# PRBonn/semantic_suma

Measured on AMD Instinct MI355X. Metric: scans_per_sec, higher is better.
Workload: dtype f32; 1 GPU; BASELINE configs[1]: synthetic KITTI-like sequence, 64x2048 range images, semantic-weighted ICP (10 GN iterations + stats pass) + surfel fusion, one sequence per GPU, scans resident in HBM, processScan called scan after scan by the native host loop (suma_pipeline_run_scans); timed after 300 untimed scans of the same sequence (5 warm-up + pre-roll to the steady map size: 1016645 surfels at the star; preroll_scans=300, map_surfels_start=1016645, map_surfels_end=2308753, parallelism=single GPU

## Files before the change

semantic_suma_amd/csrc/k_update.hip:

```cpp
#include <cstddef>
#include <cstring>

#include "suma_internal.h"

#define ST_AGG 1u
#define ST_INC 2u

__device__ __forceinline__ unsigned long long st_pack(uint32_t epoch, uint32_t flag, uint32_t value) {
  return ((unsigned long long)epoch << 34) | ((unsigned long long)flag << 32) | value;
}

struct Pair {
  uint32_t a, x;
};
__device__ __forceinline__ void lookback_publish(unsigned long long* __restrict__ status,
                                                 unsigned long long* __restrict__ group, uint32_t tile, uint32_t agg,
                                                 uint32_t epoch, uint32_t aggx = 0) {
  __hip_atomic_store(&status[tile], st_pack(epoch, ST_AGG, (aggx << 16) | agg), __ATOMIC_RELAXED, __HIP_MEMORY_SCOPE_AGENT);
  __hip_atomic_fetch_add(&group[tile >> 6], (1ull << 56) | ((unsigned long long)aggx << 32) | (unsigned long long)agg,
                         __ATOMIC_RELAXED, __HIP_MEMORY_SCOPE_AGENT);
}
#define SUMA_SPIN_LIMIT (1u << 26)
#ifndef LB_BATCH
#define LB_BATCH 4
#endif
template <bool PAIR>
__device__ Pair lookback_collect2(unsigned long long* __restrict__ status, unsigned long long* __restrict__ group,
                                  uint32_t tile, uint32_t epoch, int lane, uint32_t* __restrict__ fault) {
  const uint32_t g = tile >> 6;
  uint32_t sum = 0, sumx = 0;
  bool timed_out = false;
  const uint32_t j = tile & 63u;
  const bool own = (uint32_t)lane < j;
  unsigned long long ws = 0;
  if (own) ws = __hip_atomic_load(&status[(g << 6) + lane], __ATOMIC_RELAXED, __HIP_MEMORY_SCOPE_AGENT);
  for (uint32_t base = 0; base < g; base += 64u * LB_BATCH) {
    unsigned long long w[LB_BATCH];
#pragma unroll
    for (int q = 0; q < LB_BATCH; ++q) {
      const uint32_t gi = base + (uint32_t)q * 64u + (uint32_t)lane;
      w[q] = gi < g ? __hip_atomic_load(&group[gi], __ATOMIC_RELAXED, __HIP_MEMORY_SCOPE_AGENT) : (64ull << 56);
    }
#pragma unroll
    for (int q = 0; q < LB_BATCH; ++q) {
      const uint32_t gi = base + (uint32_t)q * 64u + (uint32_t)lane;
      uint32_t spins = 0;
      while ((uint32_t)(w[q] >> 56) != 64u && ++spins < SUMA_SPIN_LIMIT)
        w[q] = __hip_atomic_load(&group[gi], __ATOMIC_RELAXED, __HIP_MEMORY_SCOPE_AGENT);
      timed_out |= (spins >= SUMA_SPIN_LIMIT);
      sum += (uint32_t)(w[q] & 0xffffffffull);
      if (PAIR) sumx += (uint32_t)(w[q] >> 32) & 0xffffffu;
    }
  }
  if (own) {
    uint32_t spins = 0;
    while (((uint32_t)(ws >> 34) != (epoch & 0x3fffffffu) || ((ws >> 32) & 3ull) == 0) && ++spins < SUMA_SPIN_LIMIT)
      ws = __hip_atomic_load(&status[(g << 6) + lane], __ATOMIC_RELAXED, __HIP_MEMORY_SCOPE_AGENT);
    timed_out |= (spins >= SUMA_SPIN_LIMIT);
    sum += (uint32_t)(ws & 0xffffull);
    if (PAIR) sumx += (uint32_t)(ws >> 16) & 0xffffu;
  }
  if (timed_out) {
    atomicOr(fault, 8u);
    atomicOr(fault + (offsetof(DevState, fault_site) - offsetof(DevState, overflow)) / 4, 0x2u);
  }
  Pair r;
  r.a = (uint32_t)__builtin_amdgcn_readlane((int)wave_inclusive_scan(sum), 63);
  r.x = PAIR ? (uint32_t)__builtin_amdgcn_readlane((int)wave_inclusive_scan(sumx), 63) : 0u;
  return r;
}
__device__ __forceinline__ uint32_t lookback_collect(unsigned long long* __restrict__ status,
                                                     unsigned long long* __restrict__ group, uint32_t tile, uint32_t epoch,
                                                     int lane, uint32_t* __restrict__ fault) {
  return lookback_collect2<false>(status, group, tile, epoch, lane, fault).a;
}
__device__ uint32_t lookback_prefix(unsigned long long* __restrict__ status, unsigned long long* __restrict__ group,
                                    uint32_t tile, uint32_t agg, uint32_t epoch, int lane, uint32_t* __restrict__ fault) {
  if (lane == 0) lookback_publish(status, group, tile, agg, epoch);
  return lookback_collect(status, group, tile, epoch, lane, fault);
}

struct BlockRank {
  uint32_t rank, total;
};
#define TILE_WAVES (SUMA_TILE / 64)
__device__ __forceinline__ BlockRank block_rank(bool flag, uint32_t* s_wave ) {
  const int lane = threadIdx.x & 63, wave = threadIdx.x >> 6;
  const unsigned long long ball = __ballot(flag);
  const uint32_t below = __popcll(ball & ((1ull << lane) - 1ull));
  if (lane == 0) s_wave[wave] = __popcll(ball);
  __syncthreads();
  uint32_t off = 0, tot = 0;
#pragma unroll
  for (int w = 0; w < (int)TILE_WAVES; ++w) {
    uint32_t cnt = s_wave[w];
    if (w < wave) off += cnt;
    tot += cnt;
  }
  BlockRank r;
  r.rank = off + below;
  r.total = tot;
  return r;
}

__device__ __forceinline__ void block_rank2(bool fa, bool fb, uint32_t* s_wa, uint32_t* s_wb, BlockRank* ra, BlockRank* rb) {
  const int lane = threadIdx.x & 63, wave = threadIdx.x >> 6;
  const unsigned long long ba = __ballot(fa), bb = __ballot(fb);
  const unsigned long long lo = (1ull << lane) - 1ull;
  if (lane == 0) {
    s_wa[wave] = __popcll(ba);
    s_wb[wave] = __popcll(bb);
  }
  __syncthreads();
  uint32_t offa = 0, tota = 0, offb = 0, totb = 0;
#pragma unroll
  for (int w = 0; w < (int)TILE_WAVES; ++w) {
    const uint32_t ca = s_wa[w], cb = s_wb[w];
    if (w < wave) {
      offa += ca;
      offb += cb;
    }
    tota += ca;
    totb += cb;
  }
  ra->rank = offa + __popcll(ba & lo);
  ra->total = tota;
  rb->rank = offb + __popcll(bb & lo);
  rb->total = totb;
}

__device__ __forceinline__ bool is_finaliser(uint32_t failing_ticket, uint32_t ntiles) {
  return failing_ticket == ntiles + gridDim.x - 1;
}
__device__ __forceinline__ void finalise_tickets(DevState* ds, unsigned long long* group_next, uint32_t group_words) {
  for (uint32_t gi = threadIdx.x; gi < group_words; gi += blockDim.x) group_next[gi] = 0;
  if (threadIdx.x == 0) ds->ticket = 0;
}

__device__ __forceinline__ void commit_extraction(DevState* ds, CacheSlot* slots, uint32_t slot, uint32_t base,
                                                  uint32_t arena_cap, uint32_t n) {
  if (n > SUMA_EXTRACT_CAPACITY) {
    n = SUMA_EXTRACT_CAPACITY;
    atomicOr(&ds->overflow, 4u);
  }
  if ((uint64_t)base + n > arena_cap) {
    n = arena_cap - base;
    atomicOr(&ds->overflow, 2u);
  }
  slots[slot].offset = base;
  slots[slot].count = n;
  ds->cache_used = base + n;
  ds->n_extracted = n;
}

__device__ __forceinline__ void write_pose_entry(float* poses, float* poses_inv, uint32_t pose_idx, const m4& pose) {
  float inv[16];
  rigid_inverse_dev(pose.m, inv);
  for (int i = 0; i < 16; ++i) {
    poses[16 * (size_t)pose_idx + i] = pose.m[i];
    poses_inv[16 * (size_t)pose_idx + i] = inv[i];
  }
}
__global__ void __launch_bounds__(256)
    k8_radius(const float4* __restrict__ V, const float4* __restrict__ N, K8Out o, uint32_t P, DevState* ds,
              float* poses, float* poses_inv, uint32_t pose_idx, m4 pose, const float4* __restrict__ Sem) {
  uint32_t pix = blockIdx.x * blockDim.x + threadIdx.x;
  if (pix >= P) return;
  if (pix == 0) {
    ds->n_updated = 0;
    ds->n_data = 0;
    ds->n_kept_updated = 0;
    ds->n_kept_data = 0;
    write_pose_entry(poses, poses_inv, pose_idx, pose);
  }
  k8_pixel(o, pix, V[pix], N[pix], Sem[pix]);
}
__global__ void k8_pose_only(float* poses, float* poses_inv, uint32_t pose_idx, m4 pose) {
  if (threadIdx.x == 0 && blockIdx.x == 0) write_pose_entry(poses, poses_inv, pose_idx, pose);
}

struct UpdArgs {
  const suma_surfel* in;
  suma_surfel* out;
  DevState* ds;
  const float* poses;
  const float* poses_inv;
  unsigned long long* zbuf;
  unsigned long long* status;
  unsigned long long *group, *group_next;
  uint32_t group_words;
  uint32_t epoch;
  const float4 *V, *N, *Sem;
  const float4* radius_conf;
  const float4* pixrec;
  uint8_t* integrated;
  uint32_t* index_map;
  proj_t q;
  m4 pose, inv_pose;
  int32_t timestamp;
  uint32_t max_surfels;
  float confidence_threshold, map_max_distance, update_angle_thresh;
  float p_stable, p_unstable, log_prior, log_unstable, sigma_angle, sigma_distance, max_weight;
  int32_t use_stability, unstable_age, confidence_mode, active_timestamps, weighting_scheme, averaging_scheme,
      update_always;
  float cx, cy, extent;
  uint8_t* ex_flags;
  float ex_cx, ex_cy, ex_extent;
  suma_surfel* x_arena;
  CacheSlot* x_slots;
  uint32_t x_cap, x_slot;
  float* poses_w;
  float* poses_inv_w;
  uint32_t pose_idx;
  int write_pose;
};

__device__ __forceinline__ void load_pose(const float* __restrict__ table, int32_t idx, float* M) {
  const float4* src = reinterpret_cast<const float4*>(table + 16 * (size_t)idx);
#pragma unroll
  for (int k = 0; k < 4; ++k) {
    float4 col = src[k];
    M[4 * k] = col.x;
    M[4 * k + 1] = col.y;
    M[4 * k + 2] = col.z;
    M[4 * k + 3] = col.w;
  }
}

__global__ void __launch_bounds__(256) k7_indexmap(UpdArgs a) {
  const uint32_t S = a.ds->n_surfels;
  const float4* __restrict__ sf = reinterpret_cast<const float4*>(a.in);
  for (uint32_t i = blockIdx.x * blockDim.x + threadIdx.x; i < S; i += gridDim.x * blockDim.x) {
    float4 s0 = sf[4 * (size_t)i], s1 = sf[4 * (size_t)i + 1];
    float count = sf[4 * (size_t)i + 2].w;
    float Ps[16], M[16];
    load_pose(a.poses, (int32_t)count, Ps);
    m4_mul(a.inv_pose.m, Ps, M);
    v3 p = m4_point(M, xyz(s0)), n = m4_dir(M, xyz(s1));
    float lp = len3(p);
    if (!(dot3(n, divs3(neg3(p), lp)) > 0.01f)) continue;
    v3 pr = project01(a.q, p);
    float fx = sdm_floor(pr.x * a.q.width), fy = sdm_floor(pr.y * a.q.height);
    if (!(fx >= 0.0f && fx < a.q.width && fy >= 0.0f && fy < a.q.height)) continue;
    float zn = 2.0f * pr.z - 1.0f;
    if (!(zn >= -1.0f && zn <= 1.0f)) continue;
    unsigned long long key = ((unsigned long long)depth24(0.5f * zn + 0.5f) << 32) | i;
    zbuf_min(&a.zbuf[(size_t)(int32_t)fy * a.q.W + (size_t)(int32_t)fx], key);
  }
}

__device__ __forceinline__ v3 slerp3(v3 v0, v3 v1, float weight) {
  float omega = sdm_acos(dot3(normalize3(v0), normalize3(v1)));
  float so = sdm_sin(omega);
  if (!(so > 0.0f)) return v0;
  float eta = 1.0f / so;
  float w0 = eta * sdm_sin(weight * omega);
  float w1 = eta * sdm_sin((1.0f - weight) * omega);
  return add3(scale3(w0, v0), scale3(w1, v1));
}

struct Surfel4 {
  float4 a, b, c, d;
};

__device__ __forceinline__ bool in_active_area(const UpdArgs& a, const Surfel4& s, bool* in_tile) {
  float Ps[16];
  load_pose(a.poses, (int32_t)s.c.w, Ps);
  v3 pos = m4_point(Ps, xyz(s.a));
  *in_tile = !(sdm_abs(pos.x - a.ex_cx) > a.ex_extent || sdm_abs(pos.y - a.ex_cy) > a.ex_extent);
  if ((int32_t)__float_as_uint(s.c.x) < 0) return false;
  if (sdm_abs(pos.x - a.cx) > a.extent || sdm_abs(pos.y - a.cy) > a.extent) return false;
  return true;
}

__device__ __forceinline__ void store_surfel(suma_surfel* out, uint32_t idx, const Surfel4& s) {
  float4* o = reinterpret_cast<float4*>(out) + 4 * (size_t)idx;
  store_stream(o, s.a);
  store_stream(o + 1, s.b);
  store_stream(o + 2, s.c);
  store_stream(o + 3, s.d);
}

struct K9Pre {
  v3 old_position, old_normal;
  float imz;
  int32_t tx, ty;
  uint32_t rpix;
  bool in_tex, visible, inside;
};
struct K9Rec {
  float4 dv, dn, dx;
  unsigned long long k7key;
};

__device__ __forceinline__ K9Pre k9_prepare(const UpdArgs& a, const Surfel4& in) {
  K9Pre p;
  const int32_t creation_timestamp = (int32_t)in.c.w;
  float Ps[16];
  load_pose(a.poses, creation_timestamp, Ps);
  p.old_position = m4_point(Ps, xyz(in.a));
  p.old_normal = m4_dir(Ps, xyz(in.b));
  const v3 vertex = m4_point(a.inv_pose.m, p.old_position);
  const v3 normal = normalize3(m4_dir(a.inv_pose.m, p.old_normal));
  p.visible = dot3(normal, divs3(neg3(vertex), len3(vertex))) > 0.0f;
  const v3 pr = project01(a.q, vertex);
  const float imx = sdm_floor(pr.x * a.q.width) + 0.5f, imy = sdm_floor(pr.y * a.q.height) + 0.5f;
  p.imz = pr.z;
  p.in_tex = (imx >= 0.0f && imx < a.q.width && imy >= 0.0f && imy < a.q.height);
  p.tx = p.in_tex ? (int32_t)sdm_floor(imx) : -1;
  p.ty = p.in_tex ? (int32_t)sdm_floor(imy) : -1;
  p.rpix = (uint32_t)max(p.ty, 0) * (uint32_t)a.q.W + (uint32_t)max(p.tx, 0);
  p.inside = (imx < a.q.width && imy < a.q.height && p.imz < 1.0f) && !(imx < 0.0f && imy < 0.0f && p.imz < 0.0f);
  return p;
}

__device__ __forceinline__ K9Rec k9_gather(const UpdArgs& a, const K9Pre& p) {
  K9Rec r;
  const float4* __restrict__ rec = a.pixrec + 4 * (size_t)p.rpix;
  r.dv = rec[0];
  r.dn = rec[1];
  r.dx = rec[2];
  r.k7key = a.zbuf[p.rpix];
  return r;
}

__device__ __forceinline__ bool k9_finish(const UpdArgs& a, uint32_t i, const Surfel4& in, const K9Pre& p,
                                          const K9Rec& g, Surfel4& o, int32_t* mark_pix) {
  const int32_t timestamp = a.timestamp;
  const int32_t W = a.q.W;
  const int32_t surfel_age = timestamp - (int32_t)__float_as_uint(in.c.x);
  const int32_t creation_timestamp = (int32_t)in.c.w;
  const v3 old_position = p.old_position, old_normal = p.old_normal;
  const float old_radius = in.a.w, old_confidence = in.b.w, old_weight = in.c.z;

  bool keep = true;
  if (old_confidence < a.confidence_threshold && a.use_stability) keep = (surfel_age < a.unstable_age);
  o = in;
  o.c.y = pack_rgb(0.3f, 0.3f, 0.3f);

  float4 dv = g.dv, dn = g.dn, dx = g.dx;
  if (!p.in_tex) dv = dn = dx = f4(0.f, 0.f, 0.f, 0.f);
  const float4 ds = f4(dx.x, 0.f, 0.f, dx.y), rc = f4(dx.z, 0.f, 0.f, 0.f);
  const unsigned long long k7key = g.k7key;
  const bool valid = (dv.w > 0.5f) && (dn.w > 0.5f);
  const float imz = p.imz;
  const int32_t tx = p.tx, ty = p.ty;

  float penalty = 0.0f;
  float update_confidence = a.log_prior;
  bool mark = false;

  if (valid && p.inside && p.visible) {
    const float data_label = ds.x * 255.0f, data_prob = ds.w;
    const float model_label = in.d.x * 255.0f, model_prob = in.d.w;
    if (sdm_round(data_label) != sdm_round(model_label)) {
      if (is_dynamic_label(model_label)) penalty = 1.0f;
    }
    const v3 v = xyz(dv), n = xyz(dn);
    const v3 v_global = m4_point(a.pose.m, v);
    const v3 n_global = normalize3(m4_dir(a.pose.m, n));
    const v3 view_dir = divs3(neg3(v), len3(v));
    const float distance = sdm_abs(dot3(old_normal, sub3(v_global, old_position)));
    const float angle = len3(cross3(n_global, old_normal));
    const float new_radius = rc.x, new_confidence = rc.y;

    if ((distance < a.map_max_distance) && (angle < a.update_angle_thresh)) {
      mark = true;
      const float confidence = old_confidence + new_confidence;
      o.b.w = confidence;
      o.c.x = __uint_as_float((uint32_t)timestamp);
      float avg_radius = fmin_(new_radius, old_radius);
      avg_radius = fmax_(avg_radius, 0.0f);
      o.a.w = avg_radius;
      keep = true;
      o.c.y = pack_rgb(0.0f, 0.7f, 0.0f);
      o.c.w = (float)creation_timestamp;

      float pst = a.p_stable;
      if (a.confidence_mode == 1 || a.confidence_mode == 3)
        pst *= sdm_exp((-angle * angle) / (a.sigma_angle * a.sigma_angle));
      if (a.confidence_mode == 2 || a.confidence_mode == 3)
        pst *= sdm_exp((-distance * distance) / (a.sigma_distance * a.sigma_distance));
      pst = fclamp(pst, a.p_unstable, 1.0f);
      update_confidence = sdm_log(pst / (1.0f - pst));

      if ((new_radius < old_radius && timestamp - creation_timestamp < a.active_timestamps) || a.update_always) {
        float w1 = 0.9f, w2 = 0.1f;
        if (a.weighting_scheme > 0) {
          w1 = old_weight;
          w2 = 1.0f;
          if (a.weighting_scheme == 2) w2 = dot3(n, view_dir);
          o.c.z = fmin_(a.max_weight, w1 + w2);
          float sum = w1 + w2;
          w1 /= sum;
          w2 /= sum;
        }
        v3 avg_position = add3(scale3(w1, old_position), scale3(w2, v_global));
        v3 avg_normal = slerp3(old_normal, n_global, w1);
        float avg_prob;
        if (sdm_round(data_label) != sdm_round(model_label))
          avg_prob = w1 * model_prob + w2 * (1.0f - data_prob);
        else
          avg_prob = w1 * model_prob + w2 * data_prob;
        o.d.w = avg_prob;
        if (a.averaging_scheme == 1) {
          avg_position = add3(old_position, scale3(w2 * distance, old_normal));
          avg_normal = slerp3(old_normal, n_global, w1);
        }
        avg_normal = normalize3(avg_normal);
        float Pi[16];
        load_pose(a.poses_inv, creation_timestamp, Pi);
        avg_position = m4_point(Pi, avg_position);
        avg_normal = m4_dir(Pi, avg_normal);
        o.a = f4(avg_position.x, avg_position.y, avg_position.z, avg_radius);
        o.b = f4(avg_normal.x, avg_normal.y, avg_normal.z, confidence);
        o.c.y = pack_rgb(1.0f, 0.0f, 1.0f);
      }
    } else {
      int32_t idx = (k7key == SUMA_EMPTY_KEY) ? -1 : (int32_t)(uint32_t)(k7key & 0xffffffffull);
      if (idx == (int32_t)i) {
        update_confidence = sdm_log(a.p_unstable / (1.0f - a.p_unstable));
        o.c.y = pack_rgb(0.0f, 1.0f, 1.0f);
      }
    }
  }
  update_confidence = update_confidence - penalty;
  if (a.use_stability)
    o.b.w = fmin_((old_confidence + update_confidence) - a.log_prior, 20.0f);
  else
    o.b.w = old_confidence;
  if (o.b.w < a.log_unstable && a.use_stability) keep = false;

  *mark_pix = -1;
  if (keep && mark) {
    float zn = 2.0f * imz - 1.0f;
    if (zn >= -1.0f && zn <= 1.0f) *mark_pix = ty * W + tx;
  }
  return keep;
}

#ifndef K9_PER
#define K9_PER 1
#endif
#define K9_THREADS (SUMA_TILE / K9_PER)
#define K9_WAVES (K9_THREADS / 64)
static_assert(SUMA_TILE % K9_PER == 0 && K9_THREADS <= 1024, "K9 tile split");

__device__ __forceinline__ Surfel4 load_surfel(const float4* __restrict__ sf, uint32_t i) {
  Surfel4 r;
  r.a = sf[4 * (size_t)i];
  r.b = sf[4 * (size_t)i + 1];
  r.c = sf[4 * (size_t)i + 2];
  r.d = sf[4 * (size_t)i + 3];
  return r;
}

#if defined(__HIP_DEVICE_COMPILE__) && !defined(UPD_NO_ARG_RELOAD)
#define UPD_ARG_RELOAD 1
#endif
#ifdef UPD_ARG_RELOAD
typedef const UpdArgs __attribute__((address_space(4))) * UpdArgsK;
__device__ __forceinline__ UpdArgsK upd_args_again(UpdArgsK p) {
  asm volatile("" : "+s"(p));
  return p;
}
#endif

#ifdef SUMA_PHASE_TIMING
__device__ unsigned long long g_k9_phase[PH_BLOCKS][9];
extern "C" int suma_debug_k9_phases(unsigned long long* host, int reset) {
  hipError_t e = hipMemcpyFromSymbol(host, HIP_SYMBOL(g_k9_phase), sizeof(g_k9_phase));
  if (e == hipSuccess && reset) {
    void* p = nullptr;
    e = hipGetSymbolAddress(&p, HIP_SYMBOL(g_k9_phase));
    if (e == hipSuccess) e = hipMemset(p, 0, sizeof(g_k9_phase));
  }
  return (int)e;
}
#endif

#ifndef K9_DEFER
#define K9_DEFER 1
#endif
#define K9_BUFS (K9_DEFER ? 2 : 1)
template <bool XF>
__global__ void __launch_bounds__(K9_THREADS)
#if !K9_DEFER
    __attribute__((amdgpu_waves_per_eu(2 * K9_WAVES / 4, 2 * K9_WAVES / 4)))
#endif
    k9_update(UpdArgs a) {
  __shared__ float4 s_out[K9_BUFS][SUMA_TILE][4];
  __shared__ uint16_t s_slot[K9_BUFS][SUMA_TILE];
  __shared__ uint8_t s_ext[K9_BUFS][SUMA_TILE];
  __shared__ uint16_t s_xrank[XF ? K9_BUFS : 1][XF ? SUMA_TILE : 1];
  __shared__ uint32_t s_cnt_emit[K9_PER][K9_WAVES], s_cnt_keep[K9_WAVES], s_cnt_x[K9_PER][K9_WAVES];
  __shared__ uint32_t s_tile, s_prefix, s_prefix_x;
  const uint32_t xbase = XF ? a.ds->cache_used : 0u;
  float4* __restrict__ xdst4 = reinterpret_cast<float4*>(a.x_arena);
  const uint32_t S = a.ds->n_surfels;
  const uint32_t ntiles = (S + SUMA_TILE - 1) / SUMA_TILE;
  const float4* __restrict__ sf = reinterpret_cast<const float4*>(a.in);
  float4* __restrict__ dst4 = reinterpret_cast<float4*>(a.out);
  const int lane = threadIdx.x & 63, wave = threadIdx.x >> 6;
  uint32_t keep_count = 0;
  if (a.write_pose && blockIdx.x == 0 && threadIdx.x == 0) write_pose_entry(a.poses_w, a.poses_inv_w, a.pose_idx, a.pose);
  uint32_t prev_tile = 0xffffffffu, prev_total = 0, prev_totalx = 0, buf = 0;
#ifdef UPD_ARG_RELOAD
  const UpdArgsK ka = (UpdArgsK)__builtin_amdgcn_kernarg_segment_ptr();
#endif
  auto stream_out = [&](uint32_t pb, uint32_t tile_id, uint32_t count, uint32_t countx) {
    const uint32_t prefix = s_prefix, prefix_x = XF ? s_prefix_x : 0u;
    for (uint32_t c = threadIdx.x; c < 4u * count; c += K9_THREADS) {
      const uint64_t d = 4ull * prefix + c;
      if (d < 4ull * a.max_surfels) {
        const uint32_t slot = s_slot[pb][c >> 2];
        const float4 v = s_out[pb][slot][c & 3u];
        store_stream(&dst4[d], v);
        if (XF) {
          if (s_ext[pb][slot]) {
            const uint32_t xr = prefix_x + s_xrank[pb][slot];
            if (xr < SUMA_EXTRACT_CAPACITY && (uint64_t)xbase + xr < a.x_cap)
              store_stream(&xdst4[4ull * ((uint64_t)xbase + xr) + (c & 3u)], v);
          }
        } else if (a.ex_flags != nullptr && (c & 3u) == 0) {
          a.ex_flags[d >> 2] = s_ext[pb][slot];
        }
      }
    }
    if (tile_id == ntiles - 1 && threadIdx.x == 0) {
      const uint32_t tot = prefix + count;
      a.ds->n_kept_updated = tot < a.max_surfels ? tot : a.max_surfels;
      if (XF) a.ds->n_ext_update = prefix_x + countx;
    }
  };
  PH_BEGIN;
  for (;;) {
    PH(7);
    lds_barrier();
    if (threadIdx.x == 0)
      s_tile = __hip_atomic_fetch_add(&a.ds->ticket, 1u, __ATOMIC_RELAXED, __HIP_MEMORY_SCOPE_AGENT);
    lds_barrier();
    const uint32_t tile = s_tile;
    PH(0);
    uint32_t total = 0, totalx = 0;
    if (tile < ntiles) {
      uint32_t idx[K9_PER];
      bool live[K9_PER], emit[K9_PER];
      Surfel4 in[K9_PER];
      K9Pre pre[K9_PER];
      K9Rec rec[K9_PER];
#pragma unroll
      for (int u = 0; u < K9_PER; ++u) {
        idx[u] = tile * SUMA_TILE + (uint32_t)u * K9_THREADS + threadIdx.x;
        live[u] = idx[u] < S;
        in[u] = load_surfel(sf, live[u] ? idx[u] : 0u);
      }
#ifdef UPD_ARG_RELOAD
      const UpdArgs aA = *upd_args_again(ka);
#else
      const UpdArgs& aA = a;
#endif
#pragma unroll
      for (int u = 0; u < K9_PER; ++u) pre[u] = k9_prepare(aA, in[u]);
#ifdef SUMA_PHASE_TIMING
      if (__float_as_uint(in[0].a.x) == 0x7fc12345u) ph_acc[7] += 1;
#endif
      PH(1);
#pragma unroll
      for (int u = 0; u < K9_PER; ++u) rec[u] = k9_gather(aA, pre[u]);
#ifdef UPD_ARG_RELOAD
      const UpdArgs aB = *upd_args_again(ka);
#else
      const UpdArgs& aB = a;
#endif
      uint32_t kept = 0;
      unsigned long long eb[K9_PER], xb[K9_PER];
      bool xt[K9_PER];
#pragma unroll
      for (int u = 0; u < K9_PER; ++u) {
        Surfel4 o;
        int32_t mark_pix;
        const bool keep = k9_finish(aB, idx[u], in[u], pre[u], rec[u], o, &mark_pix) && live[u];
        if (keep && mark_pix >= 0) aB.integrated[mark_pix] = 1;
        bool in_tile;
        emit[u] = in_active_area(aB, o, &in_tile) && keep;
        const uint32_t slot = (uint32_t)u * K9_THREADS + threadIdx.x;
        xt[u] = in_tile && emit[u];
        xb[u] = XF ? __ballot(xt[u]) : 0ull;
        s_ext[buf][slot] = in_tile ? 1 : 0;
        s_out[buf][slot][0] = o.a;
        s_out[buf][slot][1] = o.b;
        s_out[buf][slot][2] = o.c;
        s_out[buf][slot][3] = o.d;
        eb[u] = __ballot(emit[u]);
        kept += __popcll(__ballot(keep));
      }
      PH(2);
      if (lane == 0) {
        s_cnt_keep[wave] = kept;
#pragma unroll
        for (int u = 0; u < K9_PER; ++u) {
          s_cnt_emit[u][wave] = __popcll(eb[u]);
          if (XF) s_cnt_x[u][wave] = __popcll(xb[u]);
        }
      }
      lds_barrier();
      uint32_t kc = 0, base = 0, basex = 0;
      const unsigned long long below = (1ull << lane) - 1ull;
#pragma unroll
      for (int u = 0; u < K9_PER; ++u) {
        uint32_t off = 0, tot = 0;
#pragma unroll
        for (int w = 0; w < K9_WAVES; ++w) {
          const uint32_t cnt = s_cnt_emit[u][w];
          if (w < wave) off += cnt;
          tot += cnt;
        }
        if (emit[u]) s_slot[buf][base + off + __popcll(eb[u] & below)] = (uint16_t)((uint32_t)u * K9_THREADS + threadIdx.x);
        base += tot;
        if (XF) {
          uint32_t offx = 0, totx = 0;
#pragma unroll
          for (int w = 0; w < K9_WAVES; ++w) {
            const uint32_t cnt = s_cnt_x[u][w];
            if (w < wave) offx += cnt;
            totx += cnt;
          }
          if (xt[u]) s_xrank[buf][(uint32_t)u * K9_THREADS + threadIdx.x] = (uint16_t)(basex + offx + __popcll(xb[u] & below));
          basex += totx;
        }
      }
#pragma unroll
      for (int w = 0; w < K9_WAVES; ++w) kc += s_cnt_keep[w];
      total = base;
      totalx = basex;
      if (threadIdx.x == 0) {
        keep_count += kc;
        lookback_publish(a.status, a.group, tile, total, a.epoch, totalx);
      }
      PH(3);
    }
    if (prev_tile != 0xffffffffu) {
      if (threadIdx.x < 64) {
        const Pair pre = lookback_collect2<XF>(a.status, a.group, prev_tile, a.epoch, threadIdx.x, &a.ds->overflow);
        if (threadIdx.x == 0) {
          s_prefix = pre.a;
          if (XF) s_prefix_x = pre.x;
        }
      }
      lds_barrier();
      PH(4);
      stream_out(buf ^ 1u, prev_tile, prev_total, prev_totalx);
      PH(5);
    }
    if (tile >= ntiles) break;
    prev_tile = tile;
    prev_total = total;
    prev_totalx = totalx;
#if K9_DEFER
    buf ^= 1u;
#else
    if (threadIdx.x < 64) {
      const Pair pre = lookback_collect2<XF>(a.status, a.group, prev_tile, a.epoch, threadIdx.x, &a.ds->overflow);
      if (threadIdx.x == 0) {
        s_prefix = pre.a;
        if (XF) s_prefix_x = pre.x;
      }
    }
    lds_barrier();
    stream_out(0u, prev_tile, prev_total, prev_totalx);
    prev_tile = 0xffffffffu;
#endif
  }
  PH_END(g_k9_phase);
  if (threadIdx.x == 0 && keep_count)
    __hip_atomic_fetch_add(&a.ds->n_updated, keep_count, __ATOMIC_RELAXED, __HIP_MEMORY_SCOPE_AGENT);
  if (is_finaliser(s_tile, ntiles)) {
    finalise_tickets(a.ds, a.group_next, a.group_words);
    if (threadIdx.x == 0 && ntiles == 0) {
      a.ds->n_kept_updated = 0;
      if (XF) a.ds->n_ext_update = 0;
    }
  }
}

template <bool XF>
__global__ void __launch_bounds__(SUMA_TILE) k10_generate(UpdArgs a) {
  __shared__ uint32_t s_tile;
  __shared__ uint32_t s_wave_a[TILE_WAVES], s_wave_b[TILE_WAVES], s_wave_x[TILE_WAVES];
  __shared__ uint32_t s_prefix, s_prefix_x;
  __shared__ uint8_t s_flag[SUMA_TILE];
  __shared__ uint32_t s_rank[SUMA_TILE];
  const int32_t W = a.q.W, H = a.q.H;
  const uint32_t P = (uint32_t)W * (uint32_t)H;
  const uint32_t ntiles = (P + SUMA_TILE - 1) / SUMA_TILE;
  const uint32_t base = a.ds->n_kept_updated;
  const uint32_t xbase = XF ? a.ds->cache_used : 0u;
  const uint32_t xfirst = XF ? a.ds->n_ext_update : 0u;
  const float color = pack_rgb(0.0f, 0.0f, 1.0f);
  uint32_t new_count = 0;
#ifdef UPD_ARG_RELOAD
  const UpdArgsK ka = (UpdArgsK)__builtin_amdgcn_kernarg_segment_ptr();
#endif
  for (;;) {
    __syncthreads();
    if (threadIdx.x == 0)
      s_tile = __hip_atomic_fetch_add(&a.ds->ticket, 1u, __ATOMIC_RELAXED, __HIP_MEMORY_SCOPE_AGENT);
    __syncthreads();
    const uint32_t tile = s_tile;
    if (tile >= ntiles) break;
#ifdef UPD_ARG_RELOAD
    const UpdArgs aT = *upd_args_again(ka);
#else
    const UpdArgs& aT = a;
#endif
    const bool patch = (SUMA_TILE % (uint32_t)H) == 0;
    const uint32_t cols = patch ? SUMA_TILE / (uint32_t)H : 1u;
    uint32_t q;
    if (patch) {
      const uint32_t yy = threadIdx.x / cols, xx = threadIdx.x - yy * cols;
      q = xx * (uint32_t)H + yy;
    } else {
      q = threadIdx.x;
    }
    const uint32_t t = tile * SUMA_TILE + q;
    bool gen = false, emit = false, in_tile = false;
    Surfel4 s;
    if (t < P) {
      const int32_t x = (int32_t)(t / (uint32_t)H), y = (int32_t)(t % (uint32_t)H);
      const size_t pix = (size_t)y * W + x;
      const float4 v = aT.V[pix], n = aT.N[pix], rc = aT.radius_conf[pix];
      const unsigned long long key = aT.zbuf[pix];
      aT.index_map[pix] = (key == SUMA_EMPTY_KEY) ? 0u : (uint32_t)(key & 0xffffffffull) + 1u;
      aT.zbuf[pix] = SUMA_EMPTY_KEY;
      bool invalid = (v.w < 1.0f) || (n.w < 1.0f);
      invalid = invalid || (rc.w < 0.5f);
      const bool integrated = aT.integrated[pix] != 0;
      const v3 vv = xyz(v), nn = xyz(n);
      const v3 view_dir = divs3(neg3(vv), len3(vv));
      gen = (!invalid && !integrated && (dot3(nn, view_dir) > 0.01f));
      if (gen) {
        const v3 ng = normalize3(nn);
        const float4 sem = aT.Sem[pix];
        float conf = aT.log_prior;
        if (is_dynamic_label(sem.x * 255.0f)) conf = aT.log_prior - 0.5f;
        s.a = f4(v.x, v.y, v.z, rc.x);
        s.b = f4(ng.x, ng.y, ng.z, conf);
        s.c = f4(__uint_as_float((uint32_t)aT.timestamp), color, 1.0f, (float)aT.timestamp);
        s.d = sem;
        emit = in_active_area(aT, s, &in_tile);
      }
    }
    {
      const unsigned long long gb = __ballot(gen);
      if ((threadIdx.x & 63) == 0) s_wave_b[threadIdx.x >> 6] = __popcll(gb);
    }
    s_flag[q] = (emit ? 1 : 0) | ((XF && emit && in_tile) ? 2 : 0);
    __syncthreads();
    BlockRank br, brx;
    if (XF) {
      block_rank2((s_flag[threadIdx.x] & 1) != 0, (s_flag[threadIdx.x] & 2) != 0, s_wave_a, s_wave_x, &br, &brx);
      s_rank[threadIdx.x] = br.rank | (brx.rank << 16);
    } else {
      br = block_rank(s_flag[threadIdx.x] != 0, s_wave_a);
      brx.rank = brx.total = 0;
      s_rank[threadIdx.x] = br.rank;
    }
    if (threadIdx.x == 0)
      for (int w = 0; w < (int)TILE_WAVES; ++w) new_count += s_wave_b[w];
    if (threadIdx.x < 64) {
      if (threadIdx.x == 0) lookback_publish(aT.status, aT.group, tile, br.total, aT.epoch, brx.total);
      const Pair pre = lookback_collect2<XF>(aT.status, aT.group, tile, aT.epoch, threadIdx.x, &aT.ds->overflow);
      if (threadIdx.x == 0) {
        s_prefix = pre.a;
        if (XF) s_prefix_x = pre.x;
      }
    }
    __syncthreads();
    if (emit) {
      const uint32_t rk = s_rank[q];
      uint64_t dst = (uint64_t)base + s_prefix + (XF ? (rk & 0xffffu) : rk);
      if (dst < aT.max_surfels) {
        store_surfel(aT.out, (uint32_t)dst, s);
        if (XF) {
          if (in_tile) {
            const uint64_t xr = (uint64_t)xfirst + s_prefix_x + (rk >> 16);
            if (xr < SUMA_EXTRACT_CAPACITY && (uint64_t)xbase + xr < aT.x_cap) store_surfel(aT.x_arena, (uint32_t)(xbase + xr), s);
          }
        } else if (aT.ex_flags != nullptr) {
          aT.ex_flags[dst] = in_tile ? 1 : 0;
        }
      }
    }
    if (tile == ntiles - 1 && threadIdx.x == 0) {
      uint64_t kept = (uint64_t)s_prefix + br.total;
      uint64_t total = (uint64_t)base + kept;
      aT.ds->n_kept_data = (uint32_t)kept;
      if (total > aT.max_surfels) {
        total = aT.max_surfels;
        atomicOr(&aT.ds->overflow, 1u);
      }
      aT.ds->n_surfels = (uint32_t)total;
      if (XF) aT.ds->n_extracted = xfirst + s_prefix_x + brx.total;
    }
  }
  if (threadIdx.x == 0 && new_count)
    __hip_atomic_fetch_add(&a.ds->n_data, new_count, __ATOMIC_RELAXED, __HIP_MEMORY_SCOPE_AGENT);
  if (is_finaliser(s_tile, ntiles)) {
    finalise_tickets(a.ds, a.group_next, a.group_words);
    if (XF && threadIdx.x == 0) commit_extraction(a.ds, a.x_slots, a.x_slot, xbase, a.x_cap, a.ds->n_extracted);
  }
}

static void set_m4(m4& d, const float* s) {
  for (int i = 0; i < 16; ++i) d.m[i] = s[i];
}

static uint32_t compact_grid(suma_ctx* c, uint64_t items) {
  uint64_t blocks = (items + SUMA_TILE - 1) / SUMA_TILE;
  if (blocks > SUMA_COMPACT_BLOCKS) blocks = SUMA_COMPACT_BLOCKS;
  if (blocks < 1) blocks = 1;
  return (uint32_t)blocks;
}
static uint32_t stream_grid(suma_ctx* c, uint64_t items) {
  uint64_t blocks = (items + 255) / 256;
  if (blocks > SUMA_STREAM_BLOCKS) blocks = SUMA_STREAM_BLOCKS;
  if (blocks < 256) blocks = 256;
  return (uint32_t)blocks;
}

K8Out launch_k8_out(suma_ctx* c) {
  K8Out o;
  o.radius_conf = c->radius_conf;
  o.integrated = c->integrated;
  o.pixrec = c->pixrec;
  o.pixel_size = c->mc.pixel_size;
  o.angle_thresh = c->mc.radconf_angle_thresh;
  o.min_radius = c->p.min_radius;
  o.max_radius = c->p.max_radius;
  return o;
}

hipError_t launch_map_update(suma_ctx* c, const float* pose, const float* inv_pose, const suma_frame* f, float cx,
                             float cy, float extent, int k7_done, const float* ex, int fused_slot) {
  const uint32_t P = (uint32_t)c->P;
  const double S = (double)c->known_surfels;
  UpdArgs a;
  memset(&a, 0, sizeof(a));
  a.in = c->surfels[c->cur];
  a.out = c->surfels[c->cur ^ 1];
  a.ds = c->ds;
  a.poses = c->poses;
  a.poses_inv = c->poses_inv;
  a.poses_w = c->poses;
  a.poses_inv_w = c->poses_inv;
  a.zbuf = c->zbuf_data;
  a.status = c->tile_status;
  a.group_words = c->group_words;
  a.V = f->map[SUMA_MAP_VERTEX];
  a.N = f->map[SUMA_MAP_NORMAL];
  a.Sem = f->map[SUMA_MAP_SEMANTIC];
  a.radius_conf = c->radius_conf;
  a.pixrec = c->pixrec;
  a.integrated = c->integrated;
  a.index_map = c->index_map;
  a.q = c->pd;
  set_m4(a.pose, pose);
  set_m4(a.inv_pose, inv_pose);
  a.timestamp = (int32_t)c->timestamp;
  a.max_surfels = c->p.max_surfels;
  a.confidence_threshold = c->p.confidence_threshold;
  a.map_max_distance = c->p.map_max_distance;
  a.update_angle_thresh = c->mc.update_angle_thresh;
  a.p_stable = c->p.p_stable;
  a.p_unstable = c->mc.p_unstable;
  a.log_prior = c->mc.log_prior;
  a.log_unstable = c->mc.log_unstable;
  a.sigma_angle = c->p.sigma_angle;
  a.sigma_distance = c->p.sigma_distance;
  a.max_weight = c->p.max_weight;
  a.use_stability = c->p.use_stability;
  a.unstable_age = c->p.unstable_age;
  a.confidence_mode = c->p.confidence_mode;
  a.active_timestamps = c->p.active_timestamps;
  a.weighting_scheme = c->p.weighting_scheme;
  a.averaging_scheme = c->p.averaging_scheme;
  a.update_always = c->p.update_always;
  a.cx = cx;
  a.cy = cy;
  a.extent = extent;
  a.ex_flags = (ex && fused_slot < 0) ? c->extract_flags : nullptr;
  const bool xf = ex && fused_slot >= 0;
  a.x_arena = xf ? c->cache_arena : nullptr;
  a.x_slots = c->cache_slots;
  a.x_cap = c->cache_cap;
  a.x_slot = xf ? (uint32_t)fused_slot : 0u;
  a.ex_cx = ex ? ex[0] : 0.0f;
  a.ex_cy = ex ? ex[1] : 0.0f;
  a.ex_extent = ex ? ex[2] : 0.0f;
  hipStream_t st = c->ls;
  const uint32_t gridS = stream_grid(c, (uint64_t)c->known_surfels + 2 * c->P);
  a.pose_idx = c->timestamp;
  a.write_pose = 0;
  if (c->k8_fused_frame == f && c->k8_fused_stamp == c->timestamp && c->k8_fused_params == c->params_version) {
    a.write_pose = 1;
  } else {
    ProfScope ps(c, "k8_radius", 48.0 * P);
    k8_radius<<<(P + 255) / 256, 256, 0, st>>>(a.V, a.N, launch_k8_out(c), P, c->ds, c->poses, c->poses_inv, c->timestamp,
                                                a.pose, a.Sem);
  }
  c->k8_fused_frame = nullptr;
  if (!k7_done) {
    ProfScope ps(c, "k7_indexmap", 64.0 * S + 8.0 * P);
    k7_indexmap<<<gridS, 256, 0, st>>>(a);
  }
  {
    ProfScope ps(c, "k9_update_surfels", 128.0 * S + 16.0 * P);
    a.epoch = ++c->epoch;
    a.group = c->tile_group + (size_t)(a.epoch & 1u) * c->group_words;
    a.group_next = c->tile_group + (size_t)((a.epoch + 1u) & 1u) * c->group_words;
    const uint32_t grid = compact_grid(c, (uint64_t)c->known_surfels + 2 * c->P);
    if (xf)
      k9_update<true><<<grid, K9_THREADS, 0, st>>>(a);
    else
      k9_update<false><<<grid, K9_THREADS, 0, st>>>(a);
  }
  {
    ProfScope ps(c, "k10_generate_surfels", (80.0 + 12.0) * P + 64.0 * P * 0.5);
    a.epoch = ++c->epoch;
    a.group = c->tile_group + (size_t)(a.epoch & 1u) * c->group_words;
    a.group_next = c->tile_group + (size_t)((a.epoch + 1u) & 1u) * c->group_words;
    if (xf)
      k10_generate<true><<<compact_grid(c, P), SUMA_TILE, 0, st>>>(a);
    else
      k10_generate<false><<<compact_grid(c, P), SUMA_TILE, 0, st>>>(a);
  }
  return hipGetLastError();
}

__global__ void k_set_poses(float* poses, float* poses_inv, const float* src, uint32_t first, uint32_t n) {
  uint32_t k = blockIdx.x * blockDim.x + threadIdx.x;
  if (k >= n) return;
  float m[16], inv[16];
  for (int i = 0; i < 16; ++i) m[i] = src[16 * (size_t)k + i];
  rigid_inverse_dev(m, inv);
  for (int i = 0; i < 16; ++i) {
    poses[16 * (size_t)(first + k) + i] = m[i];
    poses_inv[16 * (size_t)(first + k) + i] = inv[i];
  }
}
__global__ void k_identity_poses(float* poses, float* poses_inv, uint32_t n) {
  uint32_t k = blockIdx.x * blockDim.x + threadIdx.x;
  if (k >= n) return;
  for (int i = 0; i < 16; ++i) {
    float v = (i % 5 == 0) ? 1.0f : 0.0f;
    poses[16 * (size_t)k + i] = v;
    poses_inv[16 * (size_t)k + i] = v;
  }
}

__global__ void k_clear_keys(unsigned long long* z, uint32_t n) {
  uint32_t i = blockIdx.x * blockDim.x + threadIdx.x;
  if (i < n) z[i] = SUMA_EMPTY_KEY;
}
hipError_t launch_clear_index_zbuf(suma_ctx* c) {
  uint32_t P = (uint32_t)c->P;
  k_clear_keys<<<(P + 255) / 256, 256, 0, c->ls>>>(c->zbuf_data, P);
  return hipGetLastError();
}

hipError_t launch_set_poses(suma_ctx* c, const float* d_src, uint32_t first, uint32_t n) {
  if (n == 0) return hipSuccess;
  k_set_poses<<<(n + 255) / 256, 256, 0, c->ls>>>(c->poses, c->poses_inv, d_src, first, n);
  return hipGetLastError();
}
hipError_t launch_fill_identity_poses(suma_ctx* c) {
  uint32_t n = c->p.max_poses;
  k_identity_poses<<<(n + 255) / 256, 256, 0, c->ls>>>(c->poses, c->poses_inv, n);
  return hipGetLastError();
}

struct ExtractArgs {
  const suma_surfel* in;
  suma_surfel* arena;
  DevState* ds;
  CacheSlot* slots;
  const float* poses;
  unsigned long long* status;
  unsigned long long *group, *group_next;
  uint32_t group_words;
  uint32_t epoch, slot, arena_cap;
  float cx, cy, extent;
  const uint8_t* flags;
};

#define K12_ITEMS 4u
template <bool FLAGS>
__global__ void __launch_bounds__(SUMA_TILE) k12_extract(ExtractArgs a) {
  __shared__ uint32_t s_tile, s_prefix;
  __shared__ uint32_t s_cnt[K12_ITEMS][TILE_WAVES];
  const uint32_t S = a.ds->n_surfels;
  const uint32_t span = SUMA_TILE * K12_ITEMS;
  const uint32_t ntiles = (S + span - 1) / span;
  const float4* __restrict__ sf = reinterpret_cast<const float4*>(a.in);
  const uint32_t base = a.ds->cache_used;
  const int lane = threadIdx.x & 63, wave = threadIdx.x >> 6;
  for (;;) {
    __syncthreads();
    if (threadIdx.x == 0)
      s_tile = __hip_atomic_fetch_add(&a.ds->ticket, 1u, __ATOMIC_RELAXED, __HIP_MEMORY_SCOPE_AGENT);
    __syncthreads();
    const uint32_t tile = s_tile;
    if (tile >= ntiles) break;
    float4 pa[K12_ITEMS];
    float cnt[K12_ITEMS];
    uint32_t fl[K12_ITEMS];
#pragma unroll
    for (uint32_t k = 0; k < K12_ITEMS; ++k) {
      const uint32_t i = tile * span + k * SUMA_TILE + threadIdx.x;
      pa[k] = f4(0.f, 0.f, 0.f, 0.f);
      cnt[k] = 0.f;
      fl[k] = 0;
      if (i < S) {
        if (FLAGS) {
          fl[k] = a.flags[i];
        } else {
          pa[k] = sf[4 * (size_t)i];
          cnt[k] = sf[4 * (size_t)i + 2].w;
        }
      }
    }
    bool sel[K12_ITEMS];
    uint32_t below[K12_ITEMS];
#pragma unroll
    for (uint32_t k = 0; k < K12_ITEMS; ++k) {
      const uint32_t i = tile * span + k * SUMA_TILE + threadIdx.x;
      sel[k] = false;
      if (FLAGS) {
        sel[k] = fl[k] != 0;
      } else if (i < S) {
        float Ps[16];
        load_pose(a.poses, (int32_t)cnt[k], Ps);
        v3 pos = m4_point(Ps, xyz(pa[k]));
        sel[k] = !(sdm_abs(pos.x - a.cx) > a.extent || sdm_abs(pos.y - a.cy) > a.extent);
      }
      const unsigned long long b = __ballot(sel[k]);
      below[k] = __popcll(b & ((1ull << lane) - 1ull));
      if (lane == 0) s_cnt[k][wave] = __popcll(b);
    }
    __syncthreads();
    uint32_t total = 0, rank[K12_ITEMS];
#pragma unroll
    for (uint32_t k = 0; k < K12_ITEMS; ++k) {
      uint32_t off = total;
#pragma unroll
      for (int w = 0; w < (int)TILE_WAVES; ++w) {
        const uint32_t c = s_cnt[k][w];
        if (w < wave) off += c;
        total += c;
      }
      rank[k] = off + below[k];
    }
    if (threadIdx.x < 64) {
      uint32_t pre = lookback_prefix(a.status, a.group, tile, total, a.epoch, threadIdx.x, &a.ds->overflow);
      if (threadIdx.x == 0) s_prefix = pre;
    }
    __syncthreads();
#pragma unroll
    for (uint32_t k = 0; k < K12_ITEMS; ++k) {
      if (sel[k]) {
        const uint32_t i = tile * span + k * SUMA_TILE + threadIdx.x;
        const uint32_t dst = s_prefix + rank[k];
        if (dst < SUMA_EXTRACT_CAPACITY && (uint64_t)base + dst < a.arena_cap) {
          Surfel4 s;
          s.a = FLAGS ? sf[4 * (size_t)i] : pa[k];
          s.b = sf[4 * (size_t)i + 1];
          s.c = sf[4 * (size_t)i + 2];
          s.d = sf[4 * (size_t)i + 3];
          store_surfel(a.arena, base + dst, s);
        }
      }
    }
    if (tile == ntiles - 1 && threadIdx.x == 0) a.ds->n_extracted = s_prefix + total;
  }
  if (is_finaliser(s_tile, ntiles)) {
    finalise_tickets(a.ds, a.group_next, a.group_words);
    if (threadIdx.x == 0) commit_extraction(a.ds, a.slots, a.slot, base, a.arena_cap, (ntiles == 0) ? 0u : a.ds->n_extracted);
  }
}

hipError_t launch_extract(suma_ctx* c, uint32_t slot, float cx, float cy, float extent, int use_flags) {
  ExtractArgs a;
  a.flags = use_flags ? c->extract_flags : nullptr;
  a.in = c->surfels[c->cur];
  a.arena = c->cache_arena;
  a.ds = c->ds;
  a.slots = c->cache_slots;
  a.poses = c->poses;
  a.status = c->tile_status;
  a.epoch = ++c->epoch;
  a.group_words = c->group_words;
  a.group = c->tile_group + (size_t)(a.epoch & 1u) * c->group_words;
  a.group_next = c->tile_group + (size_t)((a.epoch + 1u) & 1u) * c->group_words;
  a.slot = slot;
  a.arena_cap = c->cache_cap;
  a.cx = cx;
  a.cy = cy;
  a.extent = extent;
  ProfScope ps(c, "k12_extract_submap", (use_flags ? 1.0 : 64.0) * (double)c->known_surfels);
  const uint32_t grid = compact_grid(c, ((uint64_t)c->known_surfels + 2 * c->P + K12_ITEMS - 1) / K12_ITEMS);
  if (use_flags)
    k12_extract<true><<<grid, SUMA_TILE, 0, c->ls>>>(a);
  else
    k12_extract<false><<<grid, SUMA_TILE, 0, c->ls>>>(a);
  return hipGetLastError();
}

__global__ void __launch_bounds__(256)
    k_append_cached(suma_surfel* surfels, const suma_surfel* arena, DevState* ds, const CacheSlot* slots,
                    uint32_t slot, uint32_t max_surfels, const float* poses, uint8_t* ex_flags, float ex_cx, float ex_cy,
                    float ex_extent) {
  const CacheSlot cs = slots[slot];
  const uint32_t S = ds->n_surfels;
  const float4* __restrict__ src = reinterpret_cast<const float4*>(arena + cs.offset);
  float4* __restrict__ dst = reinterpret_cast<float4*>(surfels);
  uint32_t n = cs.count;
  if ((uint64_t)S + n > max_surfels) n = max_surfels - S;
  for (uint64_t k = (uint64_t)blockIdx.x * blockDim.x + threadIdx.x; k < 4ull * n; k += (uint64_t)gridDim.x * blockDim.x)
    dst[4ull * S + k] = src[k];
  if (ex_flags != nullptr)
    for (uint64_t k = (uint64_t)blockIdx.x * blockDim.x + threadIdx.x; k < n; k += (uint64_t)gridDim.x * blockDim.x) {
      const float4 pa = src[4 * k];
      float Ps[16];
      load_pose(poses, (int32_t)src[4 * k + 2].w, Ps);
      const v3 pos = m4_point(Ps, xyz(pa));
      ex_flags[S + k] = !(sdm_abs(pos.x - ex_cx) > ex_extent || sdm_abs(pos.y - ex_cy) > ex_extent) ? 1 : 0;
    }
}
__global__ void k_append_commit(DevState* ds, const CacheSlot* slots, uint32_t slot, uint32_t max_surfels) {
  uint32_t S = ds->n_surfels, n = slots[slot].count;
  if ((uint64_t)S + n > max_surfels) {
    n = max_surfels - S;
    atomicOr(&ds->overflow, 1u);
  }
  ds->n_surfels = S + n;
}

hipError_t launch_append_cached(suma_ctx* c, uint32_t slot) {
  float ex[3] = {0.f, 0.f, 0.f};
  if (c->flagged.valid) {
    ex[0] = (float)(2.0 * c->flagged.i * c->p.submap_extent);
    ex[1] = (float)(2.0 * c->flagged.j * c->p.submap_extent);
    ex[2] = c->p.submap_extent;
  }
  k_append_cached<<<1024, 256, 0, c->ls>>>(c->surfels[c->cur], c->cache_arena, c->ds, c->cache_slots, slot,
                                               c->p.max_surfels, c->poses, c->flagged.valid ? c->extract_flags : nullptr,
                                               ex[0], ex[1], ex[2]);
  k_append_commit<<<1, 1, 0, c->ls>>>(c->ds, c->cache_slots, slot, c->p.max_surfels);
  return hipGetLastError();
}
```

Measured before the change: 3014 scans/s.

## Defer divergent normal blending to a compacted dense pass over blending surfels

The slerp/normalize/transform of the averaged normal, which only some lanes execute, is moved out of the divergent per-surfel path. Blending surfels are compacted through LDS into a dense list, and threads then recompute the normal from the stored row and pose in a packed pass after stream_out. This is meant to cut wave divergence cost in the update kernel. It adds extra pose loads, a pixrec reload, an LDS buffer and a barrier. It also packs the dense count into the keep-count word, which relies on per-wave keep counts fitting in 8 bits.

```diff
diff --git a/semantic_suma_amd/csrc/k_update.hip b/semantic_suma_amd/csrc/k_update.hip
--- a/semantic_suma_amd/csrc/k_update.hip
+++ b/semantic_suma_amd/csrc/k_update.hip
@@ -324,8 +324,18 @@
   return r;
 }
 
+__device__ __forceinline__ v3 k9_blend_normal(v3 old_normal, v3 n_global, float w1, const float* Pi) {
+  return m4_dir(Pi, normalize3(slerp3(old_normal, n_global, w1)));
+}
+
+struct K9Aux {
+  bool compat, blend;
+  float w1;
+};
+
+template <bool DENSE>
 __device__ __forceinline__ bool k9_finish(const UpdArgs& a, uint32_t i, const Surfel4& in, const K9Pre& p,
-                                          const K9Rec& g, Surfel4& o, int32_t* mark_pix) {
+                                          const K9Rec& g, Surfel4& o, int32_t* mark_pix, K9Aux* x) {
   const int32_t timestamp = a.timestamp;
   const int32_t W = a.q.W;
   const int32_t surfel_age = timestamp - (int32_t)__float_as_uint(in.c.x);
@@ -349,6 +359,8 @@
   float penalty = 0.0f;
   float update_confidence = a.log_prior;
   bool mark = false;
+  x->compat = x->blend = false;
+  x->w1 = 0.0f;
 
   if (valid && p.inside && p.visible) {
     const float data_label = ds.x * 255.0f, data_prob = ds.w;
@@ -366,6 +378,7 @@
 
     if ((distance < a.map_max_distance) && (angle < a.update_angle_thresh)) {
       mark = true;
+      x->compat = true;
       const float confidence = old_confidence + new_confidence;
       o.b.w = confidence;
       o.c.x = __uint_as_float((uint32_t)timestamp);
@@ -396,25 +409,24 @@
           w2 /= sum;
         }
         v3 avg_position = add3(scale3(w1, old_position), scale3(w2, v_global));
-        v3 avg_normal = slerp3(old_normal, n_global, w1);
         float avg_prob;
         if (sdm_round(data_label) != sdm_round(model_label))
           avg_prob = w1 * model_prob + w2 * (1.0f - data_prob);
         else
           avg_prob = w1 * model_prob + w2 * data_prob;
         o.d.w = avg_prob;
-        if (a.averaging_scheme == 1) {
-          avg_position = add3(old_position, scale3(w2 * distance, old_normal));
-          avg_normal = slerp3(old_normal, n_global, w1);
-        }
-        avg_normal = normalize3(avg_normal);
+        if (a.averaging_scheme == 1) avg_position = add3(old_position, scale3(w2 * distance, old_normal));
         float Pi[16];
         load_pose(a.poses_inv, creation_timestamp, Pi);
         avg_position = m4_point(Pi, avg_position);
-        avg_normal = m4_dir(Pi, avg_normal);
         o.a = f4(avg_position.x, avg_position.y, avg_position.z, avg_radius);
-        o.b = f4(avg_normal.x, avg_normal.y, avg_normal.z, confidence);
+        if (!DENSE) {
+          const v3 avg_normal = k9_blend_normal(old_normal, n_global, w1, Pi);
+          o.b = f4(avg_normal.x, avg_normal.y, avg_normal.z, confidence);
+        }
         o.c.y = pack_rgb(1.0f, 0.0f, 1.0f);
+        x->blend = true;
+        x->w1 = w1;
       }
     } else {
       int32_t idx = (k7key == SUMA_EMPTY_KEY) ? -1 : (int32_t)(uint32_t)(k7key & 0xffffffffull);
@@ -437,6 +449,19 @@
     if (zn >= -1.0f && zn <= 1.0f) *mark_pix = ty * W + tx;
   }
   return keep;
+}
+
+__device__ __forceinline__ void k9_dense_normal(const UpdArgs& a, float4* row, uint32_t rpix, float w1) {
+  const float4 b = row[1];
+  const int32_t creation_timestamp = (int32_t)row[2].w;
+  float Ps[16], Pi[16];
+  load_pose(a.poses, creation_timestamp, Ps);
+  load_pose(a.poses_inv, creation_timestamp, Pi);
+  const float4 dn = a.pixrec[4 * (size_t)rpix + 1];
+  const v3 old_normal = m4_dir(Ps, xyz(b));
+  const v3 n_global = normalize3(m4_dir(a.pose.m, xyz(dn)));
+  const v3 n = k9_blend_normal(old_normal, n_global, w1, Pi);
+  row[1] = f4(n.x, n.y, n.z, b.w);
 }
 
 #ifndef K9_PER
@@ -483,6 +508,31 @@
 #define K9_DEFER 1
 #endif
 #define K9_BUFS (K9_DEFER ? 2 : 1)
+#ifndef K9_DENSE
+#define K9_DENSE 1
+#endif
+#if !K9_DEFER || K9_PER != 1
+#undef K9_DENSE
+#define K9_DENSE 0
+#endif
+
+#ifdef SUMA_PHASE_TIMING
+#define K9_WAVE_LOG_TILES 4096
+struct K9WaveLog {
+  unsigned long long arrive[K9_WAVES];
+  uint32_t lanes[K9_WAVES];
+};
+__device__ K9WaveLog g_k9_wave_log[K9_WAVE_LOG_TILES];
+extern "C" int suma_debug_k9_wave_log(void* host, int reset) {
+  hipError_t e = hipMemcpyFromSymbol(host, HIP_SYMBOL(g_k9_wave_log), sizeof(g_k9_wave_log));
+  if (e == hipSuccess && reset) {
+    void* p = nullptr;
+    e = hipGetSymbolAddress(&p, HIP_SYMBOL(g_k9_wave_log));
+    if (e == hipSuccess) e = hipMemset(p, 0, sizeof(g_k9_wave_log));
+  }
+  return (int)e;
+}
+#endif
 template <bool XF>
 __global__ void __launch_bounds__(K9_THREADS)
 #if !K9_DEFER
@@ -494,6 +544,7 @@
   __shared__ uint8_t s_ext[K9_BUFS][SUMA_TILE];
   __shared__ uint16_t s_xrank[XF ? K9_BUFS : 1][XF ? SUMA_TILE : 1];
   __shared__ uint32_t s_cnt_emit[K9_PER][K9_WAVES], s_cnt_keep[K9_WAVES], s_cnt_x[K9_PER][K9_WAVES];
+  __shared__ uint32_t s_dense[K9_DENSE ? SUMA_TILE : 1][3];
   __shared__ uint32_t s_tile, s_prefix, s_prefix_x;
   const uint32_t xbase = XF ? a.ds->cache_used : 0u;
   float4* __restrict__ xdst4 = reinterpret_cast<float4*>(a.x_arena);
@@ -542,7 +593,7 @@
     lds_barrier();
     const uint32_t tile = s_tile;
     PH(0);
-    uint32_t total = 0, totalx = 0;
+    uint32_t total = 0, totalx = 0, dense_total = 0;
     if (tile < ntiles) {
       uint32_t idx[K9_PER];
       bool live[K9_PER], emit[K9_PER];
@@ -576,11 +627,18 @@
       uint32_t kept = 0;
       unsigned long long eb[K9_PER], xb[K9_PER];
       bool xt[K9_PER];
+      bool dfr = false;
+      float dfr_w1 = 0.0f;
+      unsigned long long db = 0ull;
+#ifdef SUMA_PHASE_TIMING
+      uint32_t branch_lanes = 0;
+#endif
 #pragma unroll
       for (int u = 0; u < K9_PER; ++u) {
         Surfel4 o;
         int32_t mark_pix;
-        const bool keep = k9_finish(aB, idx[u], in[u], pre[u], rec[u], o, &mark_pix) && live[u];
+        K9Aux aux;
+        const bool keep = k9_finish<K9_DENSE != 0>(aB, idx[u], in[u], pre[u], rec[u], o, &mark_pix, &aux) && live[u];
         if (keep && mark_pix >= 0) aB.integrated[mark_pix] = 1;
         bool in_tile;
         emit[u] = in_active_area(aB, o, &in_tile) && keep;
@@ -594,18 +652,33 @@
         s_out[buf][slot][3] = o.d;
         eb[u] = __ballot(emit[u]);
         kept += __popcll(__ballot(keep));
+#if K9_DENSE
+        dfr = aux.blend && emit[u];
+        dfr_w1 = aux.w1;
+        db = __ballot(dfr);
+#endif
+#ifdef SUMA_PHASE_TIMING
+        branch_lanes += (uint32_t)__popcll(__ballot(aux.blend && keep)) | ((uint32_t)__popcll(__ballot(aux.compat && keep)) << 8);
+#endif
       }
       PH(2);
       if (lane == 0) {
-        s_cnt_keep[wave] = kept;
+        s_cnt_keep[wave] = kept | ((uint32_t)__popcll(db) << 8);
 #pragma unroll
         for (int u = 0; u < K9_PER; ++u) {
           s_cnt_emit[u][wave] = __popcll(eb[u]);
           if (XF) s_cnt_x[u][wave] = __popcll(xb[u]);
         }
+#ifdef SUMA_PHASE_TIMING
+        if (tile < K9_WAVE_LOG_TILES) {
+          g_k9_wave_log[tile].lanes[wave] = branch_lanes;
+          g_k9_wave_log[tile].arrive[wave] = wall_clock64();
+        }
+#endif
       }
       lds_barrier();
-      uint32_t kc = 0, base = 0, basex = 0;
+      uint32_t kc = 0, base = 0, basex = 0, offd = 0;
+      uint32_t rank_e[K9_PER], rank_x[K9_PER];
       const unsigned long long below = (1ull << lane) - 1ull;
 #pragma unroll
       for (int u = 0; u < K9_PER; ++u) {
@@ -616,8 +689,9 @@
           if (w < wave) off += cnt;
           tot += cnt;
         }
-        if (emit[u]) s_slot[buf][base + off + __popcll(eb[u] & below)] = (uint16_t)((uint32_t)u * K9_THREADS + threadIdx.x);
+        rank_e[u] = base + off + __popcll(eb[u] & below);
         base += tot;
+        rank_x[u] = 0;
         if (XF) {
           uint32_t offx = 0, totx = 0;
 #pragma unroll
@@ -626,18 +700,37 @@
             if (w < wave) offx += cnt;
             totx += cnt;
           }
-          if (xt[u]) s_xrank[buf][(uint32_t)u * K9_THREADS + threadIdx.x] = (uint16_t)(basex + offx + __popcll(xb[u] & below));
+          rank_x[u] = basex + offx + __popcll(xb[u] & below);
           basex += totx;
         }
       }
 #pragma unroll
-      for (int w = 0; w < K9_WAVES; ++w) kc += s_cnt_keep[w];
+      for (int w = 0; w < K9_WAVES; ++w) {
+        const uint32_t ck = s_cnt_keep[w];
+        kc += ck & 0xffu;
+        if (w < wave) offd += ck >> 8;
+        dense_total += ck >> 8;
+      }
       total = base;
       totalx = basex;
       if (threadIdx.x == 0) {
         keep_count += kc;
         lookback_publish(a.status, a.group, tile, total, a.epoch, totalx);
       }
+#pragma unroll
+      for (int u = 0; u < K9_PER; ++u) {
+        const uint32_t slot = (uint32_t)u * K9_THREADS + threadIdx.x;
+        if (emit[u]) s_slot[buf][rank_e[u]] = (uint16_t)slot;
+        if (XF && xt[u]) s_xrank[buf][slot] = (uint16_t)rank_x[u];
+      }
+#if K9_DENSE
+      if (dfr) {
+        const uint32_t e = offd + __popcll(db & below);
+        s_dense[e][0] = threadIdx.x;
+        s_dense[e][1] = pre[0].rpix;
+        s_dense[e][2] = __float_as_uint(dfr_w1);
+      }
+#endif
       PH(3);
     }
     if (prev_tile != 0xffffffffu) {
@@ -653,6 +746,22 @@
       stream_out(buf ^ 1u, prev_tile, prev_total, prev_totalx);
       PH(5);
     }
+#if K9_DENSE
+    else if (tile < ntiles)
+      lds_barrier();
+    if (tile < ntiles) {
+      const uint32_t e = K9_THREADS - 1u - threadIdx.x;
+      if (e < dense_total) {
+#ifdef UPD_ARG_RELOAD
+        const UpdArgs aC = *upd_args_again(ka);
+#else
+        const UpdArgs& aC = a;
+#endif
+        k9_dense_normal(aC, &s_out[buf][s_dense[e][0]][0], s_dense[e][1], __uint_as_float(s_dense[e][2]));
+      }
+      PH(6);
+    }
+#endif
     if (tile >= ntiles) break;
     prev_tile = tile;
     prev_total = total;
```

Result: no change. 3008 scans/s (-0.2%).
